# ZhicengShi/mclSTExp

Hardware: AMD Instinct MI355X
Metric: training spots/sec (= steps/sec x global batch) at batch 128/GPU, 224px patches, 1000 genes (higher is better)
Workload: dtype bf16

## Files before the change

### mclstexp_amd/csrc/conv3x3_rows.hip

```cpp
#include "common.h"
#include <stdlib.h>

namespace {

constexpr int CI = 128, CO = 32;
constexpr int NWAVE = 8;
constexpr int WROW = 2304 + 16;
constexpr int WF_BYTES = CO * WROW;
constexpr int SLAB_ROWS = 34;
constexpr int SLAB_BYTES = SLAB_ROWS * 256;
constexpr int FRAG_DEPTH = 1;

__device__ __forceinline__ unsigned bn_relu_pair(unsigned w, float sc0, float sc1, float sh0, float sh1) {
  return pack_bf16(fmaxf(fmaf(bf_lo(w), sc0, sh0), 0.0f), fmaxf(fmaf(bf_hi(w), sc1, sh1), 0.0f));
}

template <bool V0, bool V1, bool V2>
__device__ __forceinline__ void row_mfma(const unsigned char* __restrict__ wf, const unsigned char* __restrict__ slab,
                                         const int (&pbase)[3], f32x16& aN, f32x16& aC, f32x16& aP, u32x4 (&v)[9],
                                         const float4* __restrict__ coef4 ) {
  constexpr int D = FRAG_DEPTH, NB = D + 1;
  bf16x8 p[NB], w0[NB], w1[NB], w2[NB];
  int pb[3];
  {
    int ln = pbase[0];
    asm volatile("" : "+v"(ln));
#pragma unroll
    for (int kx = 0; kx < 3; ++kx) {
      const int i = (ln & 31) + kx;
      pb[kx] = i * 256 + ((((i & 15) ^ (ln >> 5))) << 4);
    }
  }
  auto fetch = [&](int it, int buf) {
    const int kx = it >> 3, kk = it & 7;
    p[buf] = *reinterpret_cast<const bf16x8*>(slab + (pb[kx] ^ (kk << 5)));
    if (V0) w0[buf] = *reinterpret_cast<const bf16x8*>(wf + (0 * 3 + kx) * 256 + kk * 32);
    if (V1) w1[buf] = *reinterpret_cast<const bf16x8*>(wf + (1 * 3 + kx) * 256 + kk * 32);
    if (V2) w2[buf] = *reinterpret_cast<const bf16x8*>(wf + (2 * 3 + kx) * 256 + kk * 32);

  };
#pragma unroll
  for (int it = 0; it < D; ++it) fetch(it, it % NB);
#pragma unroll
  for (int it = 0; it < 24; ++it) {
    const int cur = it % NB;
    const bool tr = it >= 12;
    const int k = tr ? (it - 12) / 3 : 0, t0 = tr ? 3 * ((it - 12) % 3) : 0;
    float4 c = make_float4(0.f, 0.f, 0.f, 0.f);
    if (tr) c = coef4[16 * k];
    const int nx = it + D, nb = nx % NB, nkx = nx >> 3, nkk = nx & 7;
    __builtin_amdgcn_sched_barrier(0);
    if (V0) aN = __builtin_amdgcn_mfma_f32_32x32x16_bf16(w0[cur], p[cur], aN, 0, 0, 0);
    if (nx < 24) {
      p[nb] = *reinterpret_cast<const bf16x8*>(slab + (pb[nkx] ^ (nkk << 5)));
      if (V0) w0[nb] = *reinterpret_cast<const bf16x8*>(wf + (0 * 3 + nkx) * 256 + nkk * 32);
    }
    if (tr) v[t0][k] = bn_relu_pair(v[t0][k], c.x, c.y, c.z, c.w);
    __builtin_amdgcn_sched_barrier(0);
    if (V1) aC = __builtin_amdgcn_mfma_f32_32x32x16_bf16(w1[cur], p[cur], aC, 0, 0, 0);
    if (nx < 24) {
      if (V1) w1[nb] = *reinterpret_cast<const bf16x8*>(wf + (1 * 3 + nkx) * 256 + nkk * 32);
    }
    if (tr) v[t0 + 1][k] = bn_relu_pair(v[t0 + 1][k], c.x, c.y, c.z, c.w);
    __builtin_amdgcn_sched_barrier(0);
    if (V2) aP = __builtin_amdgcn_mfma_f32_32x32x16_bf16(w2[cur], p[cur], aP, 0, 0, 0);
    if (nx < 24) {
      if (V2) w2[nb] = *reinterpret_cast<const bf16x8*>(wf + (2 * 3 + nkx) * 256 + nkk * 32);
    }
    if (tr) v[t0 + 2][k] = bn_relu_pair(v[t0 + 2][k], c.x, c.y, c.z, c.w);
    __builtin_amdgcn_sched_barrier(0);
  }
}

__device__ __forceinline__ void row_mfma_dispatch(int m, const unsigned char* wf, const unsigned char* slab,
                                                  const int (&pbase)[3], f32x16& aN, f32x16& aC, f32x16& aP, u32x4 (&v)[9],
                                                  const float4* coef4) {
  switch (m) {
    case 7: row_mfma<true, true, true>(wf, slab, pbase, aN, aC, aP, v, coef4); break;
    case 3: row_mfma<true, true, false>(wf, slab, pbase, aN, aC, aP, v, coef4); break;
    case 6: row_mfma<false, true, true>(wf, slab, pbase, aN, aC, aP, v, coef4); break;
    case 1: row_mfma<true, false, false>(wf, slab, pbase, aN, aC, aP, v, coef4); break;
    case 4: row_mfma<false, false, true>(wf, slab, pbase, aN, aC, aP, v, coef4); break;
    case 2: row_mfma<false, true, false>(wf, slab, pbase, aN, aC, aP, v, coef4); break;
    default: break;
  }
}


constexpr int SROW = 64;
struct RowStats {
  f32x4 gram[2], sum[2];
};

template <bool STATS>
__device__ __forceinline__ void emit_row(const f32x16& a, __amdgpu_buffer_rsrc_t orow, int ln, int x0, int W, unsigned ldo2,
                                         unsigned char* __restrict__ scratch, RowStats& st) {
  const int px = x0 + (ln & 31);
  const unsigned ooff = (unsigned)px * ldo2 + 16u * (unsigned)(ln >> 5);
  unsigned pk[8];
#pragma unroll
  for (int q = 0; q < 8; ++q) pk[q] = pack_bf16(a[2 * q], a[2 * q + 1]);
#pragma unroll
  for (int g = 0; g < 2; ++g) {
#pragma unroll
    for (int d = 0; d < 2; ++d) {
      const u32x2 r = __builtin_amdgcn_permlane32_swap(pk[4 * g + d], pk[4 * g + 2 + d], false, false);
      pk[4 * g + d] = r[0];
      pk[4 * g + 2 + d] = r[1];
    }
  }
  const u32x4 lo4 = {pk[0], pk[1], pk[2], pk[3]}, hi4 = {pk[4], pk[5], pk[6], pk[7]};
  __builtin_amdgcn_raw_buffer_store_b128(lo4, orow, ooff, 0, 0);
  __builtin_amdgcn_raw_buffer_store_b128(hi4, orow, ooff + 32u, 0, 0);
  if (STATS) {
    const bool valid = px < W;
    unsigned char* wp = scratch + (ln & 31) * SROW;
    const int wsw = ((ln & 31) >> 1) & 3, hh = ln >> 5;
    *reinterpret_cast<uint4*>(wp + ((hh ^ wsw) << 4)) = valid ? make_uint4(pk[0], pk[1], pk[2], pk[3]) : make_uint4(0u, 0u, 0u, 0u);
    *reinterpret_cast<uint4*>(wp + (((2 + hh) ^ wsw) << 4)) = valid ? make_uint4(pk[4], pk[5], pk[6], pk[7]) : make_uint4(0u, 0u, 0u, 0u);
    const int i = ln & 15, g = ln >> 4;
    const int r0 = 8 * g + (i >> 2);
    const bf16x8 ones = {0x3F80, 0x3F80, 0x3F80, 0x3F80, 0x3F80, 0x3F80, 0x3F80, 0x3F80};
#pragma unroll
    for (int cb = 0; cb < 2; ++cb) {
      const int ch = 2 * cb + ((i & 3) >> 1);
      const unsigned char* p0 = scratch + r0 * SROW + ((ch ^ ((r0 >> 1) & 3)) << 4) + (i & 1) * 8;
      const unsigned char* p1 = scratch + (r0 + 4) * SROW + ((ch ^ (((r0 + 4) >> 1) & 3)) << 4) + (i & 1) * 8;
      const v4s lo = __builtin_amdgcn_ds_read_tr16_b64_v4i16((v4s __attribute__((address_space(3)))*)p0);
      const v4s hi = __builtin_amdgcn_ds_read_tr16_b64_v4i16((v4s __attribute__((address_space(3)))*)p1);
      const bf16x8 f = {lo[0], lo[1], lo[2], lo[3], hi[0], hi[1], hi[2], hi[3]};
      st.gram[cb] = __builtin_amdgcn_mfma_f32_16x16x32_bf16(f, f, st.gram[cb], 0, 0, 0);
      st.sum[cb] = __builtin_amdgcn_mfma_f32_16x16x32_bf16(f, ones, st.sum[cb], 0, 0, 0);
    }
  }
}

__global__ __launch_bounds__(64 * NWAVE, 2) void conv3x3_fwd_rows_kernel(
    const bf16_t* __restrict__ z, int nimg, int H, int W, const float* __restrict__ gamma, const float* __restrict__ beta,
    const float* __restrict__ mean, const float* __restrict__ rstd, const bf16_t* __restrict__ W2,
    bf16_t* __restrict__ out, long long ldo, float2* __restrict__ partial, int nunits, int rc, int nchunk, int nstrip) {
  extern __shared__ __attribute__((aligned(16))) unsigned char lds[];
  const int tid = threadIdx.x, lane = tid & 63;
  const int wave = __builtin_amdgcn_readfirstlane(tid >> 6);
  const int h = lane >> 5, l31 = lane & 31;

#pragma unroll 3
  for (int g = tid; g < CO * 144; g += 64 * NWAVE) {
    const int co = g / 144, c = g - co * 144;
    *reinterpret_cast<uint4*>(lds + co * WROW + c * 16) = *reinterpret_cast<const uint4*>(W2 + (long long)g * 8);
  }
  float* coef = reinterpret_cast<float*>(lds + WF_BYTES + NWAVE * SLAB_BYTES);
  if (tid < CI) {
    const float scv = gamma[tid] * rstd[tid];
    const int quad = ((tid >> 1) & 3) * 16 + (tid >> 3);
    coef[quad * 4 + (tid & 1)] = scv;
    coef[quad * 4 + 2 + (tid & 1)] = fmaf(-mean[tid], scv, beta[tid]);
  }
  __syncthreads();

  const unsigned char* wf = lds + l31 * WROW + h * 16;
  unsigned char* slab = lds + WF_BYTES + wave * SLAB_BYTES;
  unsigned char* scratch = lds + WF_BYTES + NWAVE * SLAB_BYTES + CI * 8 + wave * (32 * SROW);
  const int pbase[3] = {lane, 0, 0};
  const unsigned row_bytes = (unsigned)W * 256u;
  const unsigned orow_bytes = (unsigned)(((long long)(W - 1) * ldo + CO) * 2);
  const unsigned ldo2 = (unsigned)(ldo * 2);

  const int total_waves = gridDim.x * NWAVE;
  for (int u = blockIdx.x * NWAVE + wave; u < nunits; u += total_waves) {
    const int strip = u % nstrip, t = u / nstrip;
    const int chunk = t % nchunk, b = t / nchunk;
    const int x0 = strip * 32;
    const int j0 = chunk * rc, j1 = min(H, j0 + rc);
    const int jin0 = max(0, j0 - 1), jin1 = min(H, j1 + 1);
    const long long img = (long long)b * H;
    u32x4 vA[9], vB[9];
    auto load_row = [&](int j, u32x4 (&v)[9]) {
      const int ln = opaque_lane(lane);
      const int xs = x0 - 1 + (ln >> 4);
      const unsigned off0 = (unsigned)(max(xs, 0) * 256 + (ln & 15) * 16);
      unsigned off1 = (unsigned)((xs + 4) * 256 + (ln & 15) * 16);
      asm volatile("" : "+v"(off1));
      const __amdgpu_buffer_rsrc_t zrow = __builtin_amdgcn_make_buffer_rsrc(
          const_cast<bf16_t*>(z) + (img + min(j, jin1 - 1)) * W * CI, 0, j < jin1 ? row_bytes : 0u, 0x00020000);
      v[0] = __builtin_amdgcn_raw_buffer_load_b128(zrow, off0, 0, 0);
#pragma unroll
      for (int tt = 1; tt < 9; ++tt) v[tt] = __builtin_amdgcn_raw_buffer_load_b128(zrow, off1 + (tt - 1) * 1024u, 0, 0);
    };
    const float4* coef4 = reinterpret_cast<const float4*>(coef) + (lane & 15);
    auto transform_row = [&](u32x4 (&v)[9]) {
#pragma unroll
      for (int k = 0; k < 4; ++k) {
        const float4 c = coef4[16 * k];
#pragma unroll
        for (int tt = 0; tt < 9; ++tt) v[tt][k] = bn_relu_pair(v[tt][k], c.x, c.y, c.z, c.w);
      }
    };
    auto write_row = [&](u32x4 (&v)[9]) {
      const int ln = opaque_lane(lane);
      const int sr = ln >> 4, cc = ln & 15, wbase = sr * 256 + ((cc ^ sr) << 4);
#pragma unroll
      for (int tt = 0; tt < 9; ++tt) {
        const int i = sr + 4 * tt, x = x0 - 1 + i;
        const bool ok = x >= 0 && x < W;
        if (i < SLAB_ROWS)
          *reinterpret_cast<uint4*>(slab + (wbase ^ ((tt & 3) << 6)) + tt * 1024) =
              ok ? make_uint4(v[tt][0], v[tt][1], v[tt][2], v[tt][3]) : make_uint4(0u, 0u, 0u, 0u);
      }
    };

    RowStats st;
#pragma unroll
    for (int cb = 0; cb < 2; ++cb)
#pragma unroll
      for (int r = 0; r < 4; ++r) st.gram[cb][r] = st.sum[cb][r] = 0.0f;
    f32x16 aP, aC, aN;
#pragma unroll
    for (int r = 0; r < 16; ++r) aP[r] = aC[r] = aN[r] = 0.0f;
    load_row(jin0, vB);
    load_row(jin0 + 1, vA);
    transform_row(vB);
    write_row(vB);
    int j = jin0;
    bool more = true;
#define MCL_STEP(X, Y)                                                                                         \
    {                                                                                                          \
      more = j + 1 < jin1;                                                                                     \
      load_row(j + 2, Y);                                                                                      \
      const int m = (j + 1 < j1 ? 1 : 0) | ((j >= j0 && j < j1) ? 2 : 0) | (j - 1 >= j0 ? 4 : 0);              \
      row_mfma_dispatch(m, wf, slab, pbase, aN, aC, aP, X, coef4);                                             \
      if ((m & 4))                                                                           \
        emit_row<true>(aP, __builtin_amdgcn_make_buffer_rsrc(out + (img + j - 1) * W * ldo, 0, orow_bytes, 0x00020000), \
                       opaque_lane(lane), x0, W, ldo2, scratch, st);                                           \
      if (j == H - 1 && (m & 2))                                                                               \
        emit_row<true>(aC, __builtin_amdgcn_make_buffer_rsrc(out + (img + j) * W * ldo, 0, orow_bytes, 0x00020000),    \
                       opaque_lane(lane), x0, W, ldo2, scratch, st);                                           \
      if (more) write_row(X);                                                                \
      aP = aC;                                                                                                 \
      aC = aN;                                                                                                 \
      _Pragma("unroll") for (int r = 0; r < 16; ++r) aN[r] = 0.0f;                                             \
      ++j;                                                                                                     \
    }
    while (true) {
      MCL_STEP(vA, vB)
      if (!more) break;
      MCL_STEP(vB, vA)
      if (!more) break;
    }
#undef MCL_STEP

    if (partial != nullptr) {
      const int i = lane & 15;
      if ((lane >> 4) == (i >> 2)) {
        const int r = i & 3;
#pragma unroll
        for (int cb = 0; cb < 2; ++cb) {
          const float q = r == 0 ? st.gram[cb][0] : r == 1 ? st.gram[cb][1] : r == 2 ? st.gram[cb][2] : st.gram[cb][3];
          const float sm = r == 0 ? st.sum[cb][0] : r == 1 ? st.sum[cb][1] : r == 2 ? st.sum[cb][2] : st.sum[cb][3];
          partial[(long long)u * CO + 16 * cb + i] = make_float2(sm, q);
        }
      }
    }

  }
}

__global__ __launch_bounds__(256) void sums_finalize_kernel(const float2* __restrict__ partial, int nunits, long long S,
                                                            float eps, float* __restrict__ mean, float* __restrict__ var,
                                                            float* __restrict__ rstd) {
  __shared__ double red[2][4];
  const int c = blockIdx.x, lane = threadIdx.x & 63, wave = threadIdx.x >> 6;
  const float2* p = partial + c;
  double sum = 0.0, q = 0.0;
  constexpr int U = 8;
  for (int t0 = threadIdx.x; t0 < nunits; t0 += 256 * U) {
    float2 v[U];
#pragma unroll
    for (int u = 0; u < U; ++u) v[u] = p[(long long)min(t0 + 256 * u, nunits - 1) * CO];
#pragma unroll
    for (int u = 0; u < U; ++u) {
      if (t0 + 256 * u >= nunits) v[u] = make_float2(0.0f, 0.0f);
      sum += (double)v[u].x;
      q += (double)v[u].y;
    }
  }
#pragma unroll
  for (int o = 32; o > 0; o >>= 1) {
    sum += __shfl_xor(sum, o, 64);
    q += __shfl_xor(q, o, 64);
  }
  if (lane == 0) {
    red[0][wave] = sum;
    red[1][wave] = q;
  }
  __syncthreads();
  if (threadIdx.x != 0) return;
  sum = (red[0][0] + red[0][1]) + (red[0][2] + red[0][3]);
  q = (red[1][0] + red[1][1]) + (red[1][2] + red[1][3]);
  const double n = (double)S, m = sum / n;
  double vv = (q - sum * sum / n) / n;
  if (vv < 0.0) vv = 0.0;
  mean[c] = (float)m;
  var[c] = (float)vv;
  rstd[c] = (float)(1.0 / sqrt(vv + (double)eps));
}

struct RowsPlan {
  int nimg, nstrip, rc, nchunk, nunits, grid;
};

inline RowsPlan rows_plan(long long S, int H, int W) {
  RowsPlan p;
  p.nimg = (int)(S / ((long long)H * W));
  p.nstrip = (W + 31) / 32;
  long long rc = ((long long)H * p.nimg * p.nstrip) / 2048;
  if (rc < 2) rc = 2;
  if (rc > H) rc = H;
  p.rc = (int)rc;
  p.nchunk = (H + p.rc - 1) / p.rc;
  p.nunits = p.nimg * p.nchunk * p.nstrip;
  p.grid = (p.nunits + NWAVE - 1) / NWAVE;
  if (p.grid > 256) p.grid = 256;
  return p;
}

}

bool mcl_conv3x3_rows_applicable(long long S, int H, int W) {
  return W >= 17 && W <= 150 && H >= 1 && S % ((long long)H * W) == 0;
}

long long mcl_conv3x3_rows_workspace_floats(long long S) {
  return (S / 16 + 8) * CO * 2;
}

int mcl_launch_conv3x3_fwd_rows(const void* z, long long S, int H, int W, const float* gamma, const float* beta,
                                const float* mean, const float* rstd, const void* W2, void* out, long long ldo,
                                float* workspace, float eps, float* ymean, float* yvar, float* yrstd, hipStream_t st) {
  const RowsPlan p = rows_plan(S, H, W);
  const size_t lds_bytes = WF_BYTES + NWAVE * SLAB_BYTES + CI * 8 + NWAVE * 32 * SROW;
  static mcl_device_once attr_once;
  if (auto attr_guard = attr_once.first()) {
    (void)hipFuncSetAttribute(reinterpret_cast<const void*>(conv3x3_fwd_rows_kernel),
                              hipFuncAttributeMaxDynamicSharedMemorySize, 160 * 1024);
  }
  float2* part = reinterpret_cast<float2*>(workspace);
  hipLaunchKernelGGL(conv3x3_fwd_rows_kernel, dim3(p.grid), dim3(64 * NWAVE), lds_bytes, st, (const bf16_t*)z, p.nimg, H, W,
                     gamma, beta, mean, rstd, (const bf16_t*)W2, (bf16_t*)out, ldo, ymean != nullptr ? part : (float2*)nullptr,
                     p.nunits, p.rc, p.nchunk, p.nstrip);
  if (ymean != nullptr)
    hipLaunchKernelGGL(sums_finalize_kernel, dim3(CO), dim3(256), 0, st, (const float2*)part, p.nunits, S, eps, ymean, yvar,
                       yrstd);
  return 0;
}
```

### mclstexp_amd/csrc/conv3x3_wrw_rows.hip

```cpp
#include "common.h"
#include <stdlib.h>

namespace {

constexpr int WR_NWAVE = 8;
constexpr int WR_MN = 32 * 9 * 128;
constexpr int WR_RED_BYTES = 4 * 9 * 16 * 64 * 4;

__device__ __forceinline__ bf16x8 wr_frag(const unsigned char* p) {
  const v4s lo = __builtin_amdgcn_ds_read_tr16_b64_v4i16((v4s __attribute__((address_space(3)))*)p);
  const v4s hi = __builtin_amdgcn_ds_read_tr16_b64_v4i16((v4s __attribute__((address_space(3)))*)(p + 256));
  return bf16x8{lo[0], lo[1], lo[2], lo[3], hi[0], hi[1], hi[2], hi[3]};
}

template <int NKS>
__global__ __launch_bounds__(64 * WR_NWAVE, 2) void conv3x3_wrw_rows_kernel(
    const bf16_t* __restrict__ dy, long long lddy, const bf16_t* __restrict__ z, int nimg, int H, int W,
    const float* __restrict__ gamma, const float* __restrict__ beta, const float* __restrict__ mean,
    const float* __restrict__ rstd, int rc, int nchunk, float* __restrict__ wpart) {
  constexpr int A2_BYTES = 16 * NKS * 64;
  constexpr int SLOT = (16 * NKS + 2) * 64;
  constexpr int WAVE_LDS = A2_BYTES + 3 * SLOT;
  constexpr int NZ = NKS, ND = NKS + 1;
  extern __shared__ __attribute__((aligned(16))) unsigned char lds[];
  const int tid = threadIdx.x, lane = tid & 63;
  const int wave = __builtin_amdgcn_readfirstlane(tid >> 6);
  const int h = lane >> 5, l31 = lane & 31;
  const int q = wave & 3, stream = wave >> 2;
  unsigned char* a2buf = lds + wave * WAVE_LDS;
  unsigned char* ring = a2buf + A2_BYTES;

  float sc[8], sh[8];
#pragma unroll
  for (int j = 0; j < 8; ++j) {
    const int c = 32 * q + 8 * (lane & 3) + j;
    sc[j] = gamma[c] * rstd[c];
    sh[j] = fmaf(-mean[c], sc[j], beta[c]);
  }

  f32x16 acc[9];
#pragma unroll
  for (int t = 0; t < 9; ++t)
#pragma unroll
    for (int r = 0; r < 16; ++r) acc[t][r] = 0.0f;

  const int la = (8 * h + ((lane & 15) >> 2)) * 64 + 32 * ((lane >> 4) & 1) + 8 * (lane & 3);
  const unsigned zrow_bytes = (unsigned)W * 256u;
  const unsigned dyrow_bytes = (unsigned)(((long long)(W - 1) * lddy + 32) * 2);
  const unsigned lddy2 = (unsigned)(lddy * 2);
  const int nunit = nimg * nchunk;
  const int ustride = gridDim.x * 2;

  for (int u = blockIdx.x * 2 + stream; u < nunit; u += ustride) {
    const int chunk = u % nchunk, b = u / nchunk;
    const int j0 = chunk * rc, j1 = min(H, j0 + rc);
    const long long img = (long long)b * H;
    auto load_z = [&](int r, u32x4 (&v)[NZ]) {
      const int ln = opaque_lane(lane);
      const __amdgpu_buffer_rsrc_t row = __builtin_amdgcn_make_buffer_rsrc(
          const_cast<bf16_t*>(z) + (img + min(r, H - 1)) * W * 128, 0, r < j1 ? zrow_bytes : 0u, 0x00020000);
      const unsigned off = (unsigned)(ln >> 2) * 256u + (unsigned)q * 64u + (unsigned)(ln & 3) * 16u;
#pragma unroll
      for (int tt = 0; tt < NZ; ++tt) v[tt] = __builtin_amdgcn_raw_buffer_load_b128(row, off + tt * 4096u, 0, 0);
    };
    auto write_a2 = [&](const u32x4 (&v)[NZ]) {
      const int ln = opaque_lane(lane);
#pragma unroll
      for (int tt = 0; tt < NZ; ++tt) {
        const int x = 16 * tt + (ln >> 2);
        unsigned w[4] = {v[tt][0], v[tt][1], v[tt][2], v[tt][3]};
#pragma unroll
        for (int d = 0; d < 4; ++d) {
          const float lo = fmaxf(fmaf(__uint_as_float(w[d] << 16), sc[2 * d], sh[2 * d]), 0.0f);
          const float hi = fmaxf(fmaf(__uint_as_float(w[d] & 0xFFFF0000u), sc[2 * d + 1], sh[2 * d + 1]), 0.0f);
          w[d] = x < W ? pack_bf16(lo, hi) : 0u;
        }
        *reinterpret_cast<uint4*>(a2buf + x * 64 + (ln & 3) * 16) = make_uint4(w[0], w[1], w[2], w[3]);
      }
    };
    auto load_dy = [&](int y, u32x4 (&d)[ND]) {
      const int ln = opaque_lane(lane);
      const bool inr = y >= 0 && y < H;
      const __amdgpu_buffer_rsrc_t row = __builtin_amdgcn_make_buffer_rsrc(
          const_cast<bf16_t*>(dy) + (img + min(max(y, 0), H - 1)) * W * lddy, 0, inr ? dyrow_bytes : 0u, 0x00020000);
#pragma unroll
      for (int tt = 0; tt < ND; ++tt) {
        const int x = 16 * tt + (ln >> 2) - 1;
        d[tt] = __builtin_amdgcn_raw_buffer_load_b128(row, (unsigned)max(x, 0) * lddy2 + (unsigned)(ln & 3) * 16u, 0, 0);
      }
    };
    auto write_dy = [&](unsigned char* slot, const u32x4 (&d)[ND]) {
      const int ln = opaque_lane(lane);
#pragma unroll
      for (int tt = 0; tt < ND; ++tt) {
        const int i = 16 * tt + (ln >> 2), x = i - 1;
        const bool ok = x >= 0 && x < W;
        if (i < 16 * NKS + 2)
          *reinterpret_cast<uint4*>(slot + i * 64 + (ln & 3) * 16) =
              ok ? make_uint4(d[tt][0], d[tt][1], d[tt][2], d[tt][3]) : make_uint4(0u, 0u, 0u, 0u);
      }
    };

    unsigned char *sA = ring, *sB = ring + SLOT, *sC = ring + 2 * SLOT;
    u32x4 zr[NZ], dr[ND];
    load_dy(j0 - 1, dr);
    load_z(j0, zr);
    write_dy(sA, dr);
    load_dy(j0, dr);
    write_a2(zr);
    write_dy(sB, dr);
    load_dy(j0 + 1, dr);
    write_dy(sC, dr);

    for (int r = j0; r < j1; ++r) {
      load_z(r + 1, zr);
      load_dy(r + 2, dr);
      __builtin_amdgcn_sched_barrier(0);
      {
        const int ln = opaque_lane(lane);
        const int lo_ = (8 * (ln >> 5) + ((ln & 15) >> 2)) * 64 + 32 * ((ln >> 4) & 1) + 8 * (ln & 3);
        const unsigned char* pa = a2buf + lo_;
        const unsigned char* p0 = sC + lo_;
        const unsigned char* p1 = sB + lo_;
        const unsigned char* p2 = sA + lo_;
#pragma unroll
        for (int ks = 0; ks < NKS; ++ks) {
          const bf16x8 fb = wr_frag(pa + ks * 1024);
          bf16x8 fa[2];
          fa[0] = wr_frag(p0 + ks * 1024 + 2 * 64);
#pragma unroll
          for (int t = 0; t < 9; ++t) {
            const int nt = t + 1;
            if (nt < 9) {
              const unsigned char* pn = (nt / 3 == 0) ? p0 : (nt / 3 == 1) ? p1 : p2;
              fa[nt & 1] = wr_frag(pn + ks * 1024 + (2 - nt % 3) * 64);
            }
            __builtin_amdgcn_sched_barrier(0);
            acc[t] = __builtin_amdgcn_mfma_f32_32x32x16_bf16(fa[t & 1], fb, acc[t], 0, 0, 0);
            __builtin_amdgcn_sched_barrier(0);
          }
        }
      }
      write_a2(zr);
      write_dy(sA, dr);
      unsigned char* t_ = sA;
      sA = sB;
      sB = sC;
      sC = t_;
    }
  }

  __syncthreads();
  float* red = reinterpret_cast<float*>(lds) + (size_t)q * (9 * 16 * 64);
  if (stream == 1) {
#pragma unroll
    for (int t = 0; t < 9; ++t)
#pragma unroll
      for (int r = 0; r < 16; ++r) red[(t * 16 + r) * 64 + lane] = acc[t][r];
  }
  __syncthreads();
  if (stream == 0) {
    float* out = wpart + (long long)blockIdx.x * WR_MN;
#pragma unroll
    for (int t = 0; t < 9; ++t)
#pragma unroll
      for (int r = 0; r < 16; ++r) {
        const int co = (r & 3) + 8 * (r >> 2) + 4 * h;
        out[(co * 9 + t) * 128 + 32 * q + l31] = acc[t][r] + red[(t * 16 + r) * 64 + lane];
      }
  }
}

struct WrwRowsPlan {
  int nimg, rc, nchunk, grid, nks;
};

inline WrwRowsPlan wrw_rows_plan(long long S, int H, int W) {
  WrwRowsPlan p;
  p.nimg = (int)(S / ((long long)H * W));
  p.nks = W <= 32 ? 2 : 4;
  const int gcap = 160;
  long long rc = ((long long)H * p.nimg + 511) / 512;
  if (rc < 1) rc = 1;
  if (rc > H) rc = H;
  p.rc = (int)rc;
  p.nchunk = (H + p.rc - 1) / p.rc;
  const int nunit = p.nimg * p.nchunk;
  p.grid = (nunit + 1) / 2;
  if (p.grid > gcap) p.grid = gcap;
  if (p.grid > 256) p.grid = 256;
  return p;
}

}

bool mcl_conv3x3_wrw_rows_applicable(long long S, int H, int W) {
  return W >= 17 && W <= 64 && S % ((long long)H * W) == 0;
}

long long mcl_conv3x3_wrw_rows_workspace_floats(long long S, int H, int W) {
  return (long long)wrw_rows_plan(S, H, W).grid * WR_MN;
}

int mcl_launch_conv3x3_wrw_rows(const void* dy, long long lddy, const void* z, long long S, int H, int W, const float* gamma,
                                const float* beta, const float* mean, const float* rstd, float* workspace, float* dW,
                                int accumulate_w, hipStream_t st) {
  const WrwRowsPlan p = wrw_rows_plan(S, H, W);
  const size_t ring_bytes = (size_t)WR_NWAVE * ((size_t)16 * p.nks * 64 + 3 * (size_t)(16 * p.nks + 2) * 64);
  const size_t lds_bytes = ring_bytes > (size_t)WR_RED_BYTES ? ring_bytes : (size_t)WR_RED_BYTES;
  static mcl_device_once attr_once;
  if (auto attr_guard = attr_once.first()) {
    (void)hipFuncSetAttribute((const void*)conv3x3_wrw_rows_kernel<2>, hipFuncAttributeMaxDynamicSharedMemorySize, 160 * 1024);
    (void)hipFuncSetAttribute((const void*)conv3x3_wrw_rows_kernel<4>, hipFuncAttributeMaxDynamicSharedMemorySize, 160 * 1024);
  }
  if (p.nks == 2)
    hipLaunchKernelGGL((conv3x3_wrw_rows_kernel<2>), dim3(p.grid), dim3(64 * WR_NWAVE), lds_bytes, st, (const bf16_t*)dy, lddy,
                       (const bf16_t*)z, p.nimg, H, W, gamma, beta, mean, rstd, p.rc, p.nchunk, workspace);
  else
    hipLaunchKernelGGL((conv3x3_wrw_rows_kernel<4>), dim3(p.grid), dim3(64 * WR_NWAVE), lds_bytes, st, (const bf16_t*)dy, lddy,
                       (const bf16_t*)z, p.nimg, H, W, gamma, beta, mean, rstd, p.rc, p.nchunk, workspace);
  mcl_launch_wrw_merge(workspace, p.grid, (long long)WR_MN, dW, accumulate_w, st);
  MCL_CHECK_LAUNCH();
  return MCL_OK;
}
```

Measured before the change: 12790.

## Prefetch next work unit's input rows across unit boundaries in conv3x3 kernels

Both the forward conv3x3 and weight-gradient kernels now decode the next work unit and issue its first input-row loads before finishing the current unit (stats write-out, loop exit). Out-of-range units get zero-size buffer resources, so the loads are harmless. In the forward kernel the first unit's loads are also issued before the weight and BN-coefficient staging into LDS, and the weight copy is batched into registers ahead of the LDS stores. The aim is to hide global-load latency at unit starts and in the prologue, at the cost of more live registers (extra dy buffers, weight chunks), which could hurt occupancy.

```diff
diff --git a/mclstexp_amd/csrc/conv3x3_rows.hip b/mclstexp_amd/csrc/conv3x3_rows.hip
--- a/mclstexp_amd/csrc/conv3x3_rows.hip
+++ b/mclstexp_amd/csrc/conv3x3_rows.hip
@@ -144,17 +144,65 @@
   const int wave = __builtin_amdgcn_readfirstlane(tid >> 6);
   const int h = lane >> 5, l31 = lane & 31;
 
-#pragma unroll 3
-  for (int g = tid; g < CO * 144; g += 64 * NWAVE) {
-    const int co = g / 144, c = g - co * 144;
-    *reinterpret_cast<uint4*>(lds + co * WROW + c * 16) = *reinterpret_cast<const uint4*>(W2 + (long long)g * 8);
+  const unsigned row_bytes = (unsigned)W * 256u;
+
+  const int total_waves = gridDim.x * NWAVE;
+  int u = blockIdx.x * NWAVE + wave;
+  int x0, j0, j1, jin0, jin1;
+  long long img;
+  unsigned live_bytes;
+  auto decode = [&](int uraw) {
+    const int uu = min(uraw, nunits - 1);
+    live_bytes = uraw < nunits ? row_bytes : 0u;
+    const int strip = uu % nstrip, t = uu / nstrip;
+    const int chunk = t % nchunk, b = t / nchunk;
+    x0 = strip * 32;
+    j0 = chunk * rc;
+    j1 = min(H, j0 + rc);
+    jin0 = max(0, j0 - 1);
+    jin1 = min(H, j1 + 1);
+    img = (long long)b * H;
+  };
+  u32x4 vA[9], vB[9];
+  auto load_row = [&](int j, u32x4 (&v)[9]) {
+    const int ln = opaque_lane(lane);
+    const int xs = x0 - 1 + (ln >> 4);
+    const unsigned off0 = (unsigned)(max(xs, 0) * 256 + (ln & 15) * 16);
+    unsigned off1 = (unsigned)((xs + 4) * 256 + (ln & 15) * 16);
+    asm volatile("" : "+v"(off1));
+    const __amdgpu_buffer_rsrc_t zrow = __builtin_amdgcn_make_buffer_rsrc(
+        const_cast<bf16_t*>(z) + (img + min(j, jin1 - 1)) * W * CI, 0, j < jin1 ? live_bytes : 0u, 0x00020000);
+    v[0] = __builtin_amdgcn_raw_buffer_load_b128(zrow, off0, 0, 0);
+#pragma unroll
+    for (int tt = 1; tt < 9; ++tt) v[tt] = __builtin_amdgcn_raw_buffer_load_b128(zrow, off1 + (tt - 1) * 1024u, 0, 0);
+  };
+
+  decode(u);
+  load_row(jin0, vB);
+  load_row(jin0 + 1, vA);
+  const int ct = tid & (CI - 1);
+  const float c_gamma = gamma[ct], c_rstd = rstd[ct], c_mean = mean[ct], c_beta = beta[ct];
+  constexpr int WCHUNKS = CO * 144 / (64 * NWAVE);
+  static_assert(WCHUNKS * 64 * NWAVE == CO * 144, "the weight copy is spelled out for exactly 9 chunks per thread");
+  u32x4 wq[WCHUNKS];
+  {
+    const __amdgpu_buffer_rsrc_t wsrc =
+        __builtin_amdgcn_make_buffer_rsrc(const_cast<bf16_t*>(W2), 0, (unsigned)(CO * 144 * 16), 0x00020000);
+#pragma unroll
+    for (int k = 0; k < WCHUNKS; ++k) wq[k] = __builtin_amdgcn_raw_buffer_load_b128(wsrc, (unsigned)(tid + k * 64 * NWAVE) * 16u, 0, 0);
+  }
+  __builtin_amdgcn_sched_barrier(0);
+#pragma unroll
+  for (int k = 0; k < WCHUNKS; ++k) {
+    const int g = tid + k * 64 * NWAVE, co = g / 144, c = g - co * 144;
+    *reinterpret_cast<u32x4*>(lds + co * WROW + c * 16) = wq[k];
   }
   float* coef = reinterpret_cast<float*>(lds + WF_BYTES + NWAVE * SLAB_BYTES);
-  if (tid < CI) {
-    const float scv = gamma[tid] * rstd[tid];
-    const int quad = ((tid >> 1) & 3) * 16 + (tid >> 3);
-    coef[quad * 4 + (tid & 1)] = scv;
-    coef[quad * 4 + 2 + (tid & 1)] = fmaf(-mean[tid], scv, beta[tid]);
+  {
+    const float scv = c_gamma * c_rstd;
+    const int quad = ((ct >> 1) & 3) * 16 + (ct >> 3);
+    coef[quad * 4 + (ct & 1)] = scv;
+    coef[quad * 4 + 2 + (ct & 1)] = fmaf(-c_mean, scv, c_beta);
   }
   __syncthreads();
 
@@ -162,32 +210,11 @@
   unsigned char* slab = lds + WF_BYTES + wave * SLAB_BYTES;
   unsigned char* scratch = lds + WF_BYTES + NWAVE * SLAB_BYTES + CI * 8 + wave * (32 * SROW);
   const int pbase[3] = {lane, 0, 0};
-  const unsigned row_bytes = (unsigned)W * 256u;
   const unsigned orow_bytes = (unsigned)(((long long)(W - 1) * ldo + CO) * 2);
   const unsigned ldo2 = (unsigned)(ldo * 2);
-
-  const int total_waves = gridDim.x * NWAVE;
-  for (int u = blockIdx.x * NWAVE + wave; u < nunits; u += total_waves) {
-    const int strip = u % nstrip, t = u / nstrip;
-    const int chunk = t % nchunk, b = t / nchunk;
-    const int x0 = strip * 32;
-    const int j0 = chunk * rc, j1 = min(H, j0 + rc);
-    const int jin0 = max(0, j0 - 1), jin1 = min(H, j1 + 1);
-    const long long img = (long long)b * H;
-    u32x4 vA[9], vB[9];
-    auto load_row = [&](int j, u32x4 (&v)[9]) {
-      const int ln = opaque_lane(lane);
-      const int xs = x0 - 1 + (ln >> 4);
-      const unsigned off0 = (unsigned)(max(xs, 0) * 256 + (ln & 15) * 16);
-      unsigned off1 = (unsigned)((xs + 4) * 256 + (ln & 15) * 16);
-      asm volatile("" : "+v"(off1));
-      const __amdgpu_buffer_rsrc_t zrow = __builtin_amdgcn_make_buffer_rsrc(
-          const_cast<bf16_t*>(z) + (img + min(j, jin1 - 1)) * W * CI, 0, j < jin1 ? row_bytes : 0u, 0x00020000);
-      v[0] = __builtin_amdgcn_raw_buffer_load_b128(zrow, off0, 0, 0);
-#pragma unroll
-      for (int tt = 1; tt < 9; ++tt) v[tt] = __builtin_amdgcn_raw_buffer_load_b128(zrow, off1 + (tt - 1) * 1024u, 0, 0);
-    };
-    const float4* coef4 = reinterpret_cast<const float4*>(coef) + (lane & 15);
+  const float4* coef4 = reinterpret_cast<const float4*>(coef) + (lane & 15);
+
+  while (u < nunits) {
     auto transform_row = [&](u32x4 (&v)[9]) {
 #pragma unroll
       for (int k = 0; k < 4; ++k) {
@@ -203,9 +230,9 @@
       for (int tt = 0; tt < 9; ++tt) {
         const int i = sr + 4 * tt, x = x0 - 1 + i;
         const bool ok = x >= 0 && x < W;
-        if (i < SLAB_ROWS)
-          *reinterpret_cast<uint4*>(slab + (wbase ^ ((tt & 3) << 6)) + tt * 1024) =
-              ok ? make_uint4(v[tt][0], v[tt][1], v[tt][2], v[tt][3]) : make_uint4(0u, 0u, 0u, 0u);
+        unsigned char* dst = slab + (wbase ^ ((tt & 3) << 6)) + tt * 1024;
+        if (4 * tt + 3 >= SLAB_ROWS) dst = i < SLAB_ROWS ? dst : scratch + (ln & 31) * 16;
+        *reinterpret_cast<uint4*>(dst) = make_uint4(ok ? v[tt][0] : 0u, ok ? v[tt][1] : 0u, ok ? v[tt][2] : 0u, ok ? v[tt][3] : 0u);
       }
     };
 
@@ -217,8 +244,6 @@
     f32x16 aP, aC, aN;
 #pragma unroll
     for (int r = 0; r < 16; ++r) aP[r] = aC[r] = aN[r] = 0.0f;
-    load_row(jin0, vB);
-    load_row(jin0 + 1, vA);
     transform_row(vB);
     write_row(vB);
     int j = jin0;
@@ -249,6 +274,12 @@
     }
 #undef MCL_STEP
 
+    const int u_done = u;
+    u += total_waves;
+    decode(u);
+    load_row(jin0, vB);
+    load_row(jin0 + 1, vA);
+
     if (partial != nullptr) {
       const int i = lane & 15;
       if ((lane >> 4) == (i >> 2)) {
@@ -257,7 +288,7 @@
         for (int cb = 0; cb < 2; ++cb) {
           const float q = r == 0 ? st.gram[cb][0] : r == 1 ? st.gram[cb][1] : r == 2 ? st.gram[cb][2] : st.gram[cb][3];
           const float sm = r == 0 ? st.sum[cb][0] : r == 1 ? st.sum[cb][1] : r == 2 ? st.sum[cb][2] : st.sum[cb][3];
-          partial[(long long)u * CO + 16 * cb + i] = make_float2(sm, q);
+          partial[(long long)u_done * CO + 16 * cb + i] = make_float2(sm, q);
         }
       }
     }
diff --git a/mclstexp_amd/csrc/conv3x3_wrw_rows.hip b/mclstexp_amd/csrc/conv3x3_wrw_rows.hip
--- a/mclstexp_amd/csrc/conv3x3_wrw_rows.hip
+++ b/mclstexp_amd/csrc/conv3x3_wrw_rows.hip
@@ -30,14 +30,6 @@
   unsigned char* a2buf = lds + wave * WAVE_LDS;
   unsigned char* ring = a2buf + A2_BYTES;
 
-  float sc[8], sh[8];
-#pragma unroll
-  for (int j = 0; j < 8; ++j) {
-    const int c = 32 * q + 8 * (lane & 3) + j;
-    sc[j] = gamma[c] * rstd[c];
-    sh[j] = fmaf(-mean[c], sc[j], beta[c]);
-  }
-
   f32x16 acc[9];
 #pragma unroll
   for (int t = 0; t < 9; ++t)
@@ -51,66 +43,85 @@
   const int nunit = nimg * nchunk;
   const int ustride = gridDim.x * 2;
 
-  for (int u = blockIdx.x * 2 + stream; u < nunit; u += ustride) {
-    const int chunk = u % nchunk, b = u / nchunk;
-    const int j0 = chunk * rc, j1 = min(H, j0 + rc);
-    const long long img = (long long)b * H;
-    auto load_z = [&](int r, u32x4 (&v)[NZ]) {
-      const int ln = opaque_lane(lane);
-      const __amdgpu_buffer_rsrc_t row = __builtin_amdgcn_make_buffer_rsrc(
-          const_cast<bf16_t*>(z) + (img + min(r, H - 1)) * W * 128, 0, r < j1 ? zrow_bytes : 0u, 0x00020000);
-      const unsigned off = (unsigned)(ln >> 2) * 256u + (unsigned)q * 64u + (unsigned)(ln & 3) * 16u;
-#pragma unroll
-      for (int tt = 0; tt < NZ; ++tt) v[tt] = __builtin_amdgcn_raw_buffer_load_b128(row, off + tt * 4096u, 0, 0);
-    };
-    auto write_a2 = [&](const u32x4 (&v)[NZ]) {
-      const int ln = opaque_lane(lane);
-#pragma unroll
-      for (int tt = 0; tt < NZ; ++tt) {
-        const int x = 16 * tt + (ln >> 2);
-        unsigned w[4] = {v[tt][0], v[tt][1], v[tt][2], v[tt][3]};
-#pragma unroll
-        for (int d = 0; d < 4; ++d) {
-          const float lo = fmaxf(fmaf(__uint_as_float(w[d] << 16), sc[2 * d], sh[2 * d]), 0.0f);
-          const float hi = fmaxf(fmaf(__uint_as_float(w[d] & 0xFFFF0000u), sc[2 * d + 1], sh[2 * d + 1]), 0.0f);
-          w[d] = x < W ? pack_bf16(lo, hi) : 0u;
-        }
-        *reinterpret_cast<uint4*>(a2buf + x * 64 + (ln & 3) * 16) = make_uint4(w[0], w[1], w[2], w[3]);
+  int u = blockIdx.x * 2 + stream;
+  int j0, j1;
+  long long img;
+  unsigned z_live, dy_live;
+  auto decode = [&](int uraw) {
+    const int uu = min(uraw, nunit - 1);
+    const int chunk = uu % nchunk, b = uu / nchunk;
+    j0 = chunk * rc;
+    j1 = min(H, j0 + rc);
+    img = (long long)b * H;
+    z_live = uraw < nunit ? zrow_bytes : 0u;
+    dy_live = uraw < nunit ? dyrow_bytes : 0u;
+  };
+  float sc[8], sh[8];
+  auto load_z = [&](int r, u32x4 (&v)[NZ]) {
+    const int ln = opaque_lane(lane);
+    const __amdgpu_buffer_rsrc_t row = __builtin_amdgcn_make_buffer_rsrc(
+        const_cast<bf16_t*>(z) + (img + min(r, H - 1)) * W * 128, 0, r < j1 ? z_live : 0u, 0x00020000);
+    const unsigned off = (unsigned)(ln >> 2) * 256u + (unsigned)q * 64u + (unsigned)(ln & 3) * 16u;
+#pragma unroll
+    for (int tt = 0; tt < NZ; ++tt) v[tt] = __builtin_amdgcn_raw_buffer_load_b128(row, off + tt * 4096u, 0, 0);
+  };
+  auto write_a2 = [&](const u32x4 (&v)[NZ]) {
+    const int ln = opaque_lane(lane);
+#pragma unroll
+    for (int tt = 0; tt < NZ; ++tt) {
+      const int x = 16 * tt + (ln >> 2);
+      unsigned w[4] = {v[tt][0], v[tt][1], v[tt][2], v[tt][3]};
+#pragma unroll
+      for (int d = 0; d < 4; ++d) {
+        const float lo = fmaxf(fmaf(__uint_as_float(w[d] << 16), sc[2 * d], sh[2 * d]), 0.0f);
+        const float hi = fmaxf(fmaf(__uint_as_float(w[d] & 0xFFFF0000u), sc[2 * d + 1], sh[2 * d + 1]), 0.0f);
+        w[d] = x < W ? pack_bf16(lo, hi) : 0u;
       }
-    };
-    auto load_dy = [&](int y, u32x4 (&d)[ND]) {
-      const int ln = opaque_lane(lane);
-      const bool inr = y >= 0 && y < H;
-      const __amdgpu_buffer_rsrc_t row = __builtin_amdgcn_make_buffer_rsrc(
-          const_cast<bf16_t*>(dy) + (img + min(max(y, 0), H - 1)) * W * lddy, 0, inr ? dyrow_bytes : 0u, 0x00020000);
-#pragma unroll
-      for (int tt = 0; tt < ND; ++tt) {
-        const int x = 16 * tt + (ln >> 2) - 1;
-        d[tt] = __builtin_amdgcn_raw_buffer_load_b128(row, (unsigned)max(x, 0) * lddy2 + (unsigned)(ln & 3) * 16u, 0, 0);
-      }
-    };
-    auto write_dy = [&](unsigned char* slot, const u32x4 (&d)[ND]) {
-      const int ln = opaque_lane(lane);
-#pragma unroll
-      for (int tt = 0; tt < ND; ++tt) {
-        const int i = 16 * tt + (ln >> 2), x = i - 1;
-        const bool ok = x >= 0 && x < W;
-        if (i < 16 * NKS + 2)
-          *reinterpret_cast<uint4*>(slot + i * 64 + (ln & 3) * 16) =
-              ok ? make_uint4(d[tt][0], d[tt][1], d[tt][2], d[tt][3]) : make_uint4(0u, 0u, 0u, 0u);
-      }
-    };
-
+      *reinterpret_cast<uint4*>(a2buf + x * 64 + (ln & 3) * 16) = make_uint4(w[0], w[1], w[2], w[3]);
+    }
+  };
+  auto load_dy = [&](int y, u32x4 (&d)[ND]) {
+    const int ln = opaque_lane(lane);
+    const bool inr = y >= 0 && y < H;
+    const __amdgpu_buffer_rsrc_t row = __builtin_amdgcn_make_buffer_rsrc(
+        const_cast<bf16_t*>(dy) + (img + min(max(y, 0), H - 1)) * W * lddy, 0, inr ? dy_live : 0u, 0x00020000);
+#pragma unroll
+    for (int tt = 0; tt < ND; ++tt) {
+      const int x = 16 * tt + (ln >> 2) - 1;
+      d[tt] = __builtin_amdgcn_raw_buffer_load_b128(row, (unsigned)max(x, 0) * lddy2 + (unsigned)(ln & 3) * 16u, 0, 0);
+    }
+  };
+  auto write_dy = [&](unsigned char* slot, const u32x4 (&d)[ND]) {
+    const int ln = opaque_lane(lane);
+#pragma unroll
+    for (int tt = 0; tt < ND; ++tt) {
+      const int i = 16 * tt + (ln >> 2), x = i - 1;
+      const bool ok = x >= 0 && x < W;
+      if (i < 16 * NKS + 2)
+        *reinterpret_cast<uint4*>(slot + i * 64 + (ln & 3) * 16) =
+            ok ? make_uint4(d[tt][0], d[tt][1], d[tt][2], d[tt][3]) : make_uint4(0u, 0u, 0u, 0u);
+    }
+  };
+
+  u32x4 zr[NZ], dr[ND], dr1[ND], dr2[ND];
+  decode(u);
+  load_dy(j0 - 1, dr);
+  load_z(j0, zr);
+  load_dy(j0, dr1);
+  load_dy(j0 + 1, dr2);
+#pragma unroll
+  for (int j = 0; j < 8; ++j) {
+    const int c = 32 * q + 8 * (lane & 3) + j;
+    sc[j] = gamma[c] * rstd[c];
+    sh[j] = fmaf(-mean[c], sc[j], beta[c]);
+  }
+
+  while (u < nunit) {
     unsigned char *sA = ring, *sB = ring + SLOT, *sC = ring + 2 * SLOT;
-    u32x4 zr[NZ], dr[ND];
-    load_dy(j0 - 1, dr);
-    load_z(j0, zr);
     write_dy(sA, dr);
-    load_dy(j0, dr);
     write_a2(zr);
-    write_dy(sB, dr);
-    load_dy(j0 + 1, dr);
-    write_dy(sC, dr);
+    write_dy(sB, dr1);
+    write_dy(sC, dr2);
 
     for (int r = j0; r < j1; ++r) {
       load_z(r + 1, zr);
@@ -148,6 +159,12 @@
       sB = sC;
       sC = t_;
     }
+    u += ustride;
+    decode(u);
+    load_dy(j0 - 1, dr);
+    load_z(j0, zr);
+    load_dy(j0, dr1);
+    load_dy(j0 + 1, dr2);
   }
 
   __syncthreads();
```

Measured after the change: 12750. About the same (-0.3%).
